# yu45020/Text_Segmentation_Image_Inpainting

Hardware: AMD Instinct MI355X
Metric: imgs/sec fwd+bwd on 512x512 partial-conv inpaint (higher is better)
Workload: dtype f32 (storage, accumulation, stencils, BatchNorm; matrix products = 6-term exact bf16 split on the bf16 MFMA, fp32-class error); 1 GPU; ImageFill 512x512 partial-conv inpainting train step (fwd+bwd, train-mode BN, L1 loss, grad all-reduce, fused SGD), 32 imgs/GPU, random line/ellipse hole masks; global_batch=32, parallelism=dp1, gemm_products=6, activation_storage=f32

## Files before the change

### text_segmentation_image_inpainting_amd/csrc/dwconv.hip

```cpp
#include "tsii_common.h"
#include "dw_lean_api.h"

#include <stdlib.h>

namespace tsii {

struct DwGeom {
    int n, h, w, c, kh, kw, sh, sw, ph, pw, dh, dw, ho, wo;
};

template <bool K3> struct DwPx { static constexpr int value = K3 ? 2 : 4; };
__device__ __forceinline__ int clampi(int v, int lo, int hi) { return v < lo ? lo : (v > hi ? hi : v); }

template <int W, bool K3>
__global__ __launch_bounds__(256) void dw_fwd_kernel(const float* __restrict__ x, const float* __restrict__ rmask,
                                                     const float* __restrict__ wT, const float* __restrict__ bias,
                                                     const float* __restrict__ denom, const float* __restrict__ keep,
                                                     DwGeom g, float* __restrict__ y) {
    constexpr int DW_PX = DwPx<K3>::value;
    const unsigned CG = (unsigned)(g.c / W);
    const unsigned nxg = (unsigned)((g.wo + DW_PX - 1) / DW_PX);
    const unsigned gx = (nxg * CG + 255u) / 256u;
    const unsigned b = xcd_remap(blockIdx.x, gridDim.x);
    const unsigned j = (b % gx) * blockDim.x + threadIdx.x;
// ... 681 lines not shown
            a.w = fmaf(vAA.w, wAA.w, fmaf(vAB.w, wAB.w, fmaf(vBA.w, wBA.w, vBB.w * wBB.w)));
            const float pmk = pls[ty * TW + tx];
            a.x = pmk != 0.f ? a.x * pmk : 0.f; a.y = pmk != 0.f ? a.y * pmk : 0.f;
            a.z = pmk != 0.f ? a.z * pmk : 0.f; a.w = pmk != 0.f ? a.w * pmk : 0.f;
            *reinterpret_cast<float4*>(out_b + (ty * w_in + tx) * c_all) = a;
            if constexpr (BNB) {
                const float4 yq = yv[k];
                const float hx = (yq.x - bmu.x) * bis.x, hy = (yq.y - bmu.y) * bis.y, hz = (yq.z - bmu.z) * bis.z, hw = (yq.w - bmu.w) * bis.w;
                const float zx = fmaf(hx, bga.x, bbe.x), zy = fmaf(hy, bga.y, bbe.y), zz = fmaf(hz, bga.z, bbe.z), zw = fmaf(hw, bga.w, bbe.w);
                const float gx = a.x * ((zx > 0.f && zx < bb.hi) ? 1.f : (zx > 0.f ? 0.f : bb.neg));
                const float gy = a.y * ((zy > 0.f && zy < bb.hi) ? 1.f : (zy > 0.f ? 0.f : bb.neg));
                const float gz = a.z * ((zz > 0.f && zz < bb.hi) ? 1.f : (zz > 0.f ? 0.f : bb.neg));
                const float gw = a.w * ((zw > 0.f && zw < bb.hi) ? 1.f : (zw > 0.f ? 0.f : bb.neg));
                vals[0] += gx; vals[1] += gy; vals[2] += gz; vals[3] += gw;
                vals[4] = fmaf(gx, hx, vals[4]); vals[5] = fmaf(gy, hy, vals[5]);
                vals[6] = fmaf(gz, hz, vals[6]); vals[7] = fmaf(gw, hw, vals[7]);
                if constexpr (DWG) {
                    float4 e = make_float4(0.f, 0.f, 0.f, 0.f);
                    if (pmk != 0.f) {
                        e.x = fminf(fmaxf(zx, zx * bb.neg), bb.hi) * pmk; e.y = fminf(fmaxf(zy, zy * bb.neg), bb.hi) * pmk;
                        e.z = fminf(fmaxf(zz, zz * bb.neg), bb.hi) * pmk; e.w = fminf(fmaxf(zw, zw * bb.neg), bb.hi) * pmk;
                    }
                    dwa[0].x = fmaf(e.x, vAA.x, dwa[0].x); dwa[0].y = fmaf(e.y, vAA.y, dwa[0].y); dwa[0].z = fmaf(e.z, vAA.z, dwa[0].z); dwa[0].w = fmaf(e.w, vAA.w, dwa[0].w);
                    dwa[1].x = fmaf(e.x, vAB.x, dwa[1].x); dwa[1].y = fmaf(e.y, vAB.y, dwa[1].y); dwa[1].z = fmaf(e.z, vAB.z, dwa[1].z); dwa[1].w = fmaf(e.w, vAB.w, dwa[1].w);
                    dwa[2].x = fmaf(e.x, vBA.x, dwa[2].x); dwa[2].y = fmaf(e.y, vBA.y, dwa[2].y); dwa[2].z = fmaf(e.z, vBA.z, dwa[2].z); dwa[2].w = fmaf(e.w, vBA.w, dwa[2].w);
                    dwa[3].x = fmaf(e.x, vBB.x, dwa[3].x); dwa[3].y = fmaf(e.y, vBB.y, dwa[3].y); dwa[3].z = fmaf(e.z, vBB.z, dwa[3].z); dwa[3].w = fmaf(e.w, vBB.w, dwa[3].w);
                }
            }
        }
        lds_barrier();
        if (more) { commit(PRO + NEW * (s + 1), NEW); commit_planes(s + 1); }
        lds_barrier();
    }
    if constexpr (BNB) {
#pragma unroll
        for (int i = 0; i < 8; ++i) {
            float v = vals[i];
            v += __shfl_xor(v, 8, 64); v += __shfl_xor(v, 16, 64); v += __shfl_xor(v, 32, 64);
            vals[i] = v;
        }
        float* mrg = ring;
        if ((threadIdx.x & 63) < CGS) {
#pragma unroll
            for (int i = 0; i < 8; ++i) mrg[((threadIdx.x >> 6) * CGS + cg) * 8 + i] = vals[i];
        }
        __syncthreads();
        if (threadIdx.x < 2 * ST_CB) {
            const int which = threadIdx.x / ST_CB, ch = threadIdx.x % ST_CB;
            if ((int)cb * ST_CB + ch < c_all) {
                float sum = 0.f;
                for (int wv = 0; wv < 4; ++wv) sum += mrg[(wv * CGS + ch / 4) * 8 + which * 4 + ch % 4];
                const int64_t prow = (n * chunks_y + cy) * strips_x + sx;
                bb.part[(prow * 2 + which) * c_all + (int)cb * ST_CB + ch] = sum;
            }
        }
    }
    if constexpr (DWG) {
        float4* m4 = reinterpret_cast<float4*>(dwm);
#pragma unroll
        for (int i = 0; i < 4; ++i) m4[i * 256 + threadIdx.x] = dwa[i];
        __syncthreads();
        const int64_t prow = (n * chunks_y + cy) * strips_x + sx;
        for (int j = threadIdx.x; j < 9 * ST_CB; j += 256) {
            const int tap = j / ST_CB, ch = j % ST_CB;
            if ((int)cb * ST_CB + ch >= c_all) continue;
            const int ky = tap / 3, kx = tap % 3;
            const int slot = (ky == 2 ? 2 : 0) + (kx == 2 ? 1 : 0);
            const int ty_sel = ky == 1 ? 0 : 1, tx_par = kx == 1 ? 0 : 1;
            float sum = 0.f;
#pragma unroll
            for (int l = 0; l < TW / 2; ++l) {
                const int ln = ty_sel * TW + 2 * l + tx_par;
                sum += dwm[((slot * 256 + ln * CGS + ch / 4) * 4) + ch % 4];
            }
            dwpart[(prow * 9 + tap) * c_all + (int)cb * ST_CB + ch] = sum;
        }
    }
}

}
#include "dw_lean.h"
#include "dw_lean_s2.h"
#include "dw_small.h"
#include "dw_rows.h"
namespace tsii {

struct StripPlan {
    bool ok;
    int chunk_rows;
    unsigned strips_x, chunks_y, cblocks;
};
#ifdef TSII_HIP_EMU
static int g_strip_target = 1536;
extern "C" void tsii_emu_set_strip_target(int v) { g_strip_target = v > 0 ? v : 1536; }
#else
#ifndef LS_TARGET
#define LS_TARGET 1536
#endif
static constexpr int g_strip_target = LS_TARGET;
#endif
static StripPlan plan_strip(int n, int hout, int wout, int c, int s, int d) {
    StripPlan p;
    p.ok = ((s == 1 && (d == 1 || d == 2 || d == 4 || d == 8)) || (s == 2 && d == 1)) && c % 4 == 0;
    p.strips_x = cdiv(wout, ST_TW / (s == 2 ? 2 : 1));
    p.cblocks = cdiv(c, ST_CB);
    const int64_t per_chunk = (int64_t)p.strips_x * p.cblocks * n;
    int64_t want = cdiv64(g_strip_target, per_chunk);
    const int max_chunks = cdiv(hout, ST_R);
    if (want > max_chunks) want = max_chunks;
    if (want < 1) want = 1;
    p.chunk_rows = cdiv(cdiv(hout, (int)want), ST_R) * ST_R;
    p.chunks_y = cdiv(hout, p.chunk_rows);
    if (per_chunk * p.chunks_y >= (1ll << 31)) p.ok = false;
    return p;
}

static inline unsigned strip_rows_per_image(const StripPlan& sp) { return sp.ok ? sp.chunks_y * sp.strips_x : 0u; }

struct FusedPlan {
    StripPlan sp;
    unsigned phases;
    bool rows_only;
};
static FusedPlan plan_fwd_strips(int n, int hout, int wout, int c, int s, int d) {
    FusedPlan fp;
    fp.rows_only = false;
    if (dw_phased_dims_ok(hout, wout, c, s, d)) {
        fp.phases = (unsigned)(d * d);
        if ((int64_t)n * d * d < (1ll << 24)) {
            fp.sp = plan_strip(n * d * d, cdiv(hout, d), cdiv(wout, d), c, 1, 1);
            return fp;
        }
    }
    fp.phases = 1u;
    fp.sp = plan_strip(n, hout, wout, c, s, d);
    if (!fp.sp.ok && dw_rows_dims_ok(hout, wout, c, s, d)) {
        fp.sp.ok = true; fp.sp.chunk_rows = hout; fp.sp.strips_x = 1; fp.sp.chunks_y = 1; fp.sp.cblocks = (unsigned)cdiv(c, ST_CB);
        fp.rows_only = true;
    }
    return fp;
}
static inline unsigned fused_rows_per_image(const FusedPlan& fp) { return fp.phases * strip_rows_per_image(fp.sp); }

static const DwBN kNoDwBN = {nullptr, nullptr, 1.f, 0.f};
static const DwBnBwd kNoBnBwd = {nullptr, nullptr, nullptr, nullptr, nullptr, 0.f, 0.f, 0.f, nullptr};

static bool dw_fused_ok(int s, int d) { return (s == 2 && d == 1) || (s == 1 && (d == 1 || d == 2 || d == 4 || d == 8)); }

#ifndef ST_DWG
#define ST_DWG 1
#endif
#ifndef SM_DWG
#define SM_DWG 1
#endif
static bool dw_dxdw_geom_ok(const DtGeom& g) {
    if (g.s != 1 || g.flip != 1 || g.pad_h < 0 || g.pad_w < 0 || g.c % 4 != 0 || dw_rows_ok(g)) return false;
    if (dw_small_ok(g)) return SM_DWG && dw_fused_ok(g.s, g.d);
    if (g.d == 1) return dw_lean_ok(g);
    return ST_DWG && (g.d == 2 || g.d == 4 || g.d == 8);
}

static int try_launch_dw_strip(const float* in, const float* pre, const float* wT, const float* bias, const float* denom,
                               const float* keep, const float* post_mul, DtGeom g, float* out, hipStream_t st,
                               DwBN ib = kNoDwBN, float* stats = nullptr, DwBnBwd bb = kNoBnBwd, float* dwpart = nullptr, bool fold = false) {
    if (g.c % 4 != 0 || !aligned16(in) || !aligned16(out) || !aligned16(wT)) return 1;
    if (ib.sc != nullptr && (!aligned16(ib.sc) || !aligned16(ib.sh))) return 1;
    const FusedPlan fp = plan_fwd_strips(g.n, g.hout, g.wout, g.c, g.s, g.d);
    const StripPlan sp = fp.sp;
    if (dwpart != nullptr && !(dw_dxdw_geom_ok(g) && sp.ok && fp.phases == 1 && !fp.rows_only && bb.y != nullptr && stats == nullptr &&
                               (ib.sc == nullptr) == !fold && denom == nullptr && keep == nullptr && bias == nullptr)) return 1;
    if (fold && dwpart == nullptr) return 1;
    const bool fused_any = ib.sc != nullptr || stats != nullptr || bb.y != nullptr;
    if (dw_rows_ok(g) && pre == nullptr && denom == nullptr && keep == nullptr && post_mul == nullptr && sp.ok &&
        (int64_t)g.n * cdiv(g.c, DR_CB) < (1ll << 31)) {
        const unsigned rcb = (unsigned)cdiv(g.c, DR_CB), rpi = fused_rows_per_image(fp);
        const dim3 rgrid((unsigned)g.n * rcb);
        if (bb.y != nullptr) hipLaunchKernelGGL((dw_rows_kernel<2>), rgrid, dim3(DR_THREADS), 0, st, in, wT, bias, g, rcb, rpi, ib, stats, bb, out);
        else if (fused_any) hipLaunchKernelGGL((dw_rows_kernel<1>), rgrid, dim3(DR_THREADS), 0, st, in, wT, bias, g, rcb, rpi, ib, stats, bb, out);
        else hipLaunchKernelGGL((dw_rows_kernel<0>), rgrid, dim3(DR_THREADS), 0, st, in, wT, bias, g, rcb, rpi, ib, stats, bb, out);
        return check_launch("dw_rows");
    }
    if (fp.rows_only) {
        TSII_REQUIRE(!fused_any, "depth-wise strips: dilation %d has a fused BatchNorm form on the row-phase kernel only (no mask planes, padding = dilation)", g.d);
        return 1;
    }
    if (dw_small_ok(g) && !(post_mul != nullptr && (denom != nullptr || keep != nullptr || bias != nullptr)) && (!fused_any || (sp.ok && dw_fused_ok(g.s, g.d))) &&
        !(fused_any && bb.y == nullptr && post_mul != nullptr)) {
        const bool dxe = denom == nullptr && keep == nullptr && bias == nullptr;
        if (bb.y == nullptr || dxe) {
            const unsigned scb = (unsigned)cdiv(g.c, SM_CB), rpi = sp.ok ? fused_rows_per_image(fp) : 1u;
            const dim3 sgrid((unsigned)g.n * scb);
#define TSII_DW_SMALL(MODE, DXE) do { \
            if (pre != nullptr) hipLaunchKernelGGL((dw_small_kernel<MODE, DXE, true>), sgrid, dim3(SM_THREADS), 0, st, in, pre, wT, bias, denom, keep, post_mul, g, scb, rpi, ib, stats, bb, out); \
            else hipLaunchKernelGGL((dw_small_kernel<MODE, DXE, false>), sgrid, dim3(SM_THREADS), 0, st, in, pre, wT, bias, denom, keep, post_mul, g, scb, rpi, ib, stats, bb, out); } while (0)
            if (bb.y != nullptr && dwpart != nullptr) {
                if (pre != nullptr) hipLaunchKernelGGL((dw_small_kernel<3, true, true>), sgrid, dim3(SM_THREADS), 0, st, in, pre, wT, bias, denom, keep, post_mul, g, scb, rpi, ib, dwpart, bb, out);
                else hipLaunchKernelGGL((dw_small_kernel<3, true, false>), sgrid, dim3(SM_THREADS), 0, st, in, pre, wT, bias, denom, keep, post_mul, g, scb, rpi, ib, dwpart, bb, out);
            }
            else if (bb.y != nullptr) TSII_DW_SMALL(2, true);
            else if (fused_any) TSII_DW_SMALL(1, false);
            else if (dxe) TSII_DW_SMALL(0, true);
            else TSII_DW_SMALL(0, false);
#undef TSII_DW_SMALL
            return check_launch("dw_small");
        }
    }
    if (!sp.ok) return 1;
    const int64_t nblk = (int64_t)sp.strips_x * sp.chunks_y * sp.cblocks * g.n * fp.phases;
    if (nblk >= (1ll << 31)) return fp.phases > 1 ? -1 : 1;
    const dim3 grid((unsigned)nblk);
    const bool fused = ib.sc != nullptr || stats != nullptr || bb.y != nullptr;
    if (!dw_fused_ok(g.s, g.d)) {
        TSII_REQUIRE(!fused, "depth-wise strips: dilation %d has a fused BatchNorm form on the row-phase kernel only (no mask planes, padding = dilation)", g.d);
        return 1;
    }
    if (bb.y != nullptr && g.s != 1) return 1;
    if (fp.phases > 1) {
        const bool takes = dw_lean_phased_ok(g) && !(post_mul != nullptr && (denom != nullptr || keep != nullptr || bias != nullptr));
        const bool dxe = denom == nullptr && keep == nullptr && bias == nullptr;
        if (!takes || (bb.y != nullptr && !dxe) || (fused && bb.y == nullptr && post_mul != nullptr)) {
            TSII_REQUIRE(!fused, "depth-wise strips: this dilated geometry has no fused BatchNorm form (input more than 2 d larger than the output per side?)");
            return 1;
        }
#define TSII_DW_LEAN_PH(MODE, DXE) do { \
            if (pre != nullptr) hipLaunchKernelGGL((dw_lean_kernel<MODE, DXE, true, true>), grid, dim3(256), 0, st, in, pre, wT, bias, denom, keep, post_mul, g, \
                                                   sp.chunk_rows, sp.strips_x, sp.chunks_y, sp.cblocks, ib, stats, bb, out); \
            else hipLaunchKernelGGL((dw_lean_kernel<MODE, DXE, false, true>), grid, dim3(256), 0, st, in, pre, wT, bias, denom, keep, post_mul, g, \
                                    sp.chunk_rows, sp.strips_x, sp.chunks_y, sp.cblocks, ib, stats, bb, out); } while (0)
        if (bb.y != nullptr) TSII_DW_LEAN_PH(2, true);
        else if (fused) TSII_DW_LEAN_PH(1, false);
        else if (dxe) TSII_DW_LEAN_PH(0, true);
        else TSII_DW_LEAN_PH(0, false);
#undef TSII_DW_LEAN_PH
        return check_launch("dw_lean_phased");
    }
    if (dw_lean_ok(g) && !(post_mul != nullptr && (denom != nullptr || keep != nullptr || bias != nullptr))) {
        const bool dxe = denom == nullptr && keep == nullptr && bias == nullptr;
#define TSII_DW_LEAN(MODE, DXE) do { \
            if (pre != nullptr) hipLaunchKernelGGL((dw_lean_kernel<MODE, DXE, true>), grid, dim3(256), 0, st, in, pre, wT, bias, denom, keep, post_mul, g, \
                                                   sp.chunk_rows, sp.strips_x, sp.chunks_y, sp.cblocks, ib, stats, bb, out); \
            else hipLaunchKernelGGL((dw_lean_kernel<MODE, DXE, false>), grid, dim3(256), 0, st, in, pre, wT, bias, denom, keep, post_mul, g, \
                                    sp.chunk_rows, sp.strips_x, sp.chunks_y, sp.cblocks, ib, stats, bb, out); } while (0)
        if (bb.y != nullptr) {
            if (!dxe) return 1;
            if (dwpart != nullptr && fold) {
                if (pre != nullptr) hipLaunchKernelGGL((dw_lean_kernel<4, true, true>), grid, dim3(256), 0, st, in, pre, wT, bias, denom, keep, post_mul, g,
                                                       sp.chunk_rows, sp.strips_x, sp.chunks_y, sp.cblocks, ib, dwpart, bb, out);
                else hipLaunchKernelGGL((dw_lean_kernel<4, true, false>), grid, dim3(256), 0, st, in, pre, wT, bias, denom, keep, post_mul, g,
                                        sp.chunk_rows, sp.strips_x, sp.chunks_y, sp.cblocks, ib, dwpart, bb, out);
                return check_launch("dw_lean (BatchNorm backward on load + dX + dW)");
            }
            if (dwpart != nullptr) {
                if (pre != nullptr) hipLaunchKernelGGL((dw_lean_kernel<3, true, true>), grid, dim3(256), 0, st, in, pre, wT, bias, denom, keep, post_mul, g,
                                                       sp.chunk_rows, sp.strips_x, sp.chunks_y, sp.cblocks, ib, dwpart, bb, out);
                else hipLaunchKernelGGL((dw_lean_kernel<3, true, false>), grid, dim3(256), 0, st, in, pre, wT, bias, denom, keep, post_mul, g,
                                        sp.chunk_rows, sp.strips_x, sp.chunks_y, sp.cblocks, ib, dwpart, bb, out);
                return check_launch("dw_lean (dX + dW)");
            }
            TSII_DW_LEAN(2, true);
        } else if (fused) {
            if (post_mul != nullptr) return 1;
            TSII_DW_LEAN(1, false);
        } else if (dxe) TSII_DW_LEAN(0, true);
        else TSII_DW_LEAN(0, false);
#undef TSII_DW_LEAN
        return check_launch("dw_lean");
    }
    if (dw_lean_s2_ok(g) && post_mul == nullptr && bb.y == nullptr) {
#define TSII_DW_LEAN_S2(MODE) do { \
            if (pre != nullptr) hipLaunchKernelGGL((dw_lean_s2_kernel<MODE, true>), grid, dim3(256), 0, st, in, pre, wT, bias, denom, keep, g, \
                                                   sp.chunk_rows, sp.strips_x, sp.chunks_y, sp.cblocks, ib, stats, out); \
            else hipLaunchKernelGGL((dw_lean_s2_kernel<MODE, false>), grid, dim3(256), 0, st, in, pre, wT, bias, denom, keep, g, \
                                    sp.chunk_rows, sp.strips_x, sp.chunks_y, sp.cblocks, ib, stats, out); } while (0)
        if (fused) TSII_DW_LEAN_S2(1);
        else TSII_DW_LEAN_S2(0);
#undef TSII_DW_LEAN_S2
        return check_launch("dw_lean_s2");
    }
#define TSII_DW_STRIP(S, D, MODE) hipLaunchKernelGGL((dw_strip_kernel<S, D, MODE>), grid, dim3(256), 0, st, in, pre, wT, bias, denom, keep, post_mul, g, \
                                                     sp.chunk_rows, sp.strips_x, sp.chunks_y, sp.cblocks, ib, stats, bb, out)
#define TSII_DW_STRIP_D(D) do { if (bb.y != nullptr && dwpart != nullptr) hipLaunchKernelGGL((dw_strip_kernel<1, D, 3>), grid, dim3(256), 0, st, in, pre, wT, bias, denom, keep, post_mul, g, \
                                                                                          sp.chunk_rows, sp.strips_x, sp.chunks_y, sp.cblocks, ib, dwpart, bb, out); \
                                else if (bb.y != nullptr) TSII_DW_STRIP(1, D, 2); else if (fused) TSII_DW_STRIP(1, D, 1); else TSII_DW_STRIP(1, D, 0); } while (0)
    if (g.s == 2 && fused) TSII_DW_STRIP(2, 1, 1);
    else if (g.s == 2) TSII_DW_STRIP(2, 1, 0);
    else if (g.d == 2) TSII_DW_STRIP_D(2);
    else if (g.d == 4) TSII_DW_STRIP_D(4);
    else if (g.d == 8) TSII_DW_STRIP_D(8);
    else if (bb.y != nullptr) hipLaunchKernelGGL((dw_strip_kernel<1, 1, 2>), grid, dim3(256), 0, st, in, pre, wT, bias, denom, keep, post_mul, g,
                                                 sp.chunk_rows, sp.strips_x, sp.chunks_y, sp.cblocks, ib, stats, bb, out);
    else if (fused) hipLaunchKernelGGL((dw_strip_kernel<1, 1, 1>), grid, dim3(256), 0, st, in, pre, wT, bias, denom, keep, post_mul, g,
                                       sp.chunk_rows, sp.strips_x, sp.chunks_y, sp.cblocks, ib, stats, bb, out);
    else hipLaunchKernelGGL((dw_strip_kernel<1, 1, 0>), grid, dim3(256), 0, st, in, pre, wT, bias, denom, keep, post_mul, g,
                            sp.chunk_rows, sp.strips_x, sp.chunks_y, sp.cblocks, ib, stats, bb, out);
    return check_launch("dw_strip");
}

#ifdef TSII_HIP_EMU
static int g_hdw_lean = 0;
extern "C" void tsii_emu_set_hdw_lean(int v) { g_hdw_lean = v; }
#define HDW_LEAN g_hdw_lean
#else
#ifndef HDW_LEAN
#define HDW_LEAN 0
#endif
#endif
bool hdw_lean_ok(int hout, int wout, int c, int s, int d) {
    if (!HDW_LEAN || !LS_ENABLE || s != 1 || c % 8 != 0 || hout < 1 || wout < 1) return false;
    if (d == 1) {
        const int64_t wmax = (int64_t)wout + 2, hmax = (int64_t)hout + 2;
        return c < (1 << 24) && hmax * wmax * 4 < (1ll << 24) && hmax * wmax * c * 4 < (1ll << 32) && (LS_ROWS * wmax + 64) * c * 4 < (1ll << 31);
    }
    if (!(d == 2 || d == 4) || wout < 8 * d || hout < 4 * d) return false;
    const int64_t wmax = (int64_t)wout + 2 * d, hmax = (int64_t)hout + 2 * d;
    return c < (1 << 24) && hmax * wmax * 4 < (1ll << 24) && hmax * wmax * c * 4 < (1ll << 32) && (LS_ROWS * wmax + 64) * c * 4 * d < (1ll << 31);
}
static FusedPlan hdw_lean_plan(int n, int hout, int wout, int c, int d) {
    FusedPlan fp;
    fp.rows_only = false;
    fp.phases = (unsigned)(d * d);
    fp.sp = plan_strip(n * d * d, cdiv(hout, d), cdiv(wout, d), c, 1, 1);
    return fp;
}
int64_t hdw_lean_rows(int n, int hout, int wout, int c, int s, int d) {
    if (!hdw_lean_ok(hout, wout, c, s, d) || (int64_t)n * d * d >= (1ll << 24)) return 0;
    const FusedPlan fp = hdw_lean_plan(n, hout, wout, c, d);
    return fp.sp.ok ? (int64_t)n * fused_rows_per_image(fp) : 0;
}
int launch_hdw_lean(const void* in, const float* w, const float* bias, int n, int hin, int win, int c, int d, int pad_h, int pad_w,
                    int hout, int wout, int flip, const float* in_sc, const float* in_sh, float in_neg, float in_hi, float* stats,
                    const void* bn_y, const float* bn_mean, const float* bn_var, const float* bn_gamma, const float* bn_beta,
                    float bn_eps, float bn_neg, float bn_hi, float* bn_part, void* out, hipStream_t st) {
    if (hdw_lean_rows(n, hout, wout, c, 1, d) <= 0) return 1;
    if (win > wout + 2 * d || hin > hout + 2 * d || pad_h < 0 || pad_w < 0) return 1;
    DtGeom g = {n, hin, win, c, 1, d, pad_h, pad_w, hout, wout, flip};
    const FusedPlan fp = hdw_lean_plan(n, hout, wout, c, d);
    const StripPlan sp = fp.sp;
    const int64_t nblk = (int64_t)sp.strips_x * sp.chunks_y * sp.cblocks * n * fp.phases;
    if (nblk >= (1ll << 31)) return 1;
    const dim3 grid((unsigned)nblk);
    const DwBN ib = {in_sc, in_sh, in_neg, in_hi};
    const DwBnBwd bb = {reinterpret_cast<const float*>(bn_y), bn_mean, bn_var, bn_gamma, bn_beta, bn_eps, bn_neg, bn_hi, bn_part};
    const float* inf = reinterpret_cast<const float*>(in);
    float* outf = reinterpret_cast<float*>(out);
    const float* none = nullptr;
#define TSII_HDW_LEAN(MODE, DXE, PHV) hipLaunchKernelGGL((dw_lean_kernel<MODE, DXE, false, PHV, true>), grid, dim3(256), 0, st, inf, none, w, bias, none, none, none, g, \
                                                         sp.chunk_rows, sp.strips_x, sp.chunks_y, sp.cblocks, ib, stats, bb, outf)
    if (bn_y != nullptr) { if (d > 1) TSII_HDW_LEAN(2, true, true); else TSII_HDW_LEAN(2, true, false); }
    else if (in_sc != nullptr || stats != nullptr) { if (d > 1) TSII_HDW_LEAN(1, false, true); else TSII_HDW_LEAN(1, false, false); }
    else { if (d > 1) TSII_HDW_LEAN(0, false, true); else TSII_HDW_LEAN(0, false, false); }
// ... 336 lines not shown
    TSII_REQUIRE(dwpart == nullptr, "dw_bwd_dxdw_bn: this geometry has no fused dX + dW form (tsii_dw_bwd_dxdw_ws_bytes() == 0)");
    TSII_REQUIRE(bb.y == nullptr, "dw_bwd_dx_bn: the BatchNorm-backward form needs a marching-strip path (tsii_dw_bwd_stat_rows() > 0)");
    const bool k3 = false;
    const int px = (vec && k3) ? DwPx<true>::value : DwPx<false>::value;
    const int64_t nblk = (int64_t)cdiv(cdiv(wd, px) * (vec ? c / 4 : c), 256) * h * n;
    TSII_REQUIRE(nblk < (1ll << 31), "dw_bwd_dx: grid limit");
    const dim3 grid((unsigned)nblk);
    if (vec && k3) hipLaunchKernelGGL((dw_bwd_dx_kernel<4, true>), grid, dim3(256), 0, st, dy, inv, ws, rmask, g, dx);
    else if (vec) hipLaunchKernelGGL((dw_bwd_dx_kernel<4, false>), grid, dim3(256), 0, st, dy, inv, ws, rmask, g, dx);
    else hipLaunchKernelGGL((dw_bwd_dx_kernel<1, false>), grid, dim3(256), 0, st, dy, inv, ws, rmask, g, dx);
    return check_launch("dw_bwd_dx");
}

extern "C" int tsii_dw_bwd_dx(const float* dy, const float* inv, const float* w, const float* rmask,
                              int n, int h, int wd, int c, int kh, int kw, int sh, int sw, int ph, int pw,
                              int dh, int dw, int ho, int wo, float* dx, float* ws, void* stream) {
    return dw_bwd_dx_impl(dy, inv, w, rmask, n, h, wd, c, kh, kw, sh, sw, ph, pw, dh, dw, ho, wo, kNoBnBwd, dx, ws, stream);
}

extern "C" int tsii_dw_bwd_dx_bn(const float* dy, const float* inv, const float* w, const float* rmask,
                                 int n, int h, int wd, int c, int kh, int kw, int sh, int sw, int ph, int pw,
                                 int dh, int dw, int ho, int wo,
                                 const float* bn_y, const float* bn_mean, const float* bn_var, const float* bn_gamma,
                                 const float* bn_beta, float bn_eps, int bn_act, float bn_slope,
                                 float* dx, float* bwd_part, float* ws, void* stream) {
    TSII_REQUIRE(bn_y && bn_mean && bn_var && bn_gamma && bn_beta && bwd_part, "dw_bwd_dx_bn: null pointer");
    TSII_REQUIRE(aligned16(bn_y) && aligned16(bn_mean) && aligned16(bn_var) && aligned16(bn_gamma) && aligned16(bn_beta),
                 "dw_bwd_dx_bn: BatchNorm operands must be 16-byte aligned");
    InBN tmp;
    TSII_REQUIRE(make_in_bn(bn_mean, bn_var, bn_act, bn_slope, &tmp) == 0, "dw_bwd_dx_bn: activation %d has no load-time form", bn_act);
    const DwBnBwd bb = {bn_y, bn_mean, bn_var, bn_gamma, bn_beta, bn_eps, tmp.neg, tmp.hi, bwd_part};
    return dw_bwd_dx_impl(dy, inv, w, rmask, n, h, wd, c, kh, kw, sh, sw, ph, pw, dh, dw, ho, wo, bb, dx, ws, stream);
}

extern "C" size_t tsii_dw_bwd_dxdw_ws_bytes(int n, int h, int wd, int c, int kh, int kw, int sh, int sw, int ph, int pw, int dh, int dw) {
    if (n <= 0 || h <= 0 || wd <= 0 || c <= 0 || c % 4 != 0 || !(kh == 3 && kw == 3 && dh == dw && dh >= 1)) return 0;
    if (sh == 2 && sw == 2 && ph == 1 && pw == 1 && dh == 1) {
        const StripPlan sp = plan_strip(n, h, wd, c, 1, 1);
        const int64_t rows = (int64_t)n * strip_rows_per_image(sp);
        if (!sp.ok || rows <= 0 || rows >= (1ll << 31) || (int64_t)sp.strips_x * sp.chunks_y * sp.cblocks * n >= (1ll << 31)) return 0;
        return (size_t)rows * 9 * (size_t)c * sizeof(float);
    }
    if (sh != 1 || sw != 1) return 0;
    const int d = dh;
    if (ph < 0 || pw < 0 || ph > 2 * d || pw > 2 * d) return 0;
    const int ho = h + 2 * ph - 2 * d, wo = wd + 2 * pw - 2 * d;
    if (ho <= 0 || wo <= 0) return 0;
    const DtGeom tg = {n, ho, wo, c, 1, d, 2 * d - ph, 2 * d - pw, h, wd, 1};
    if (!dw_dxdw_geom_ok(tg)) return 0;
    const FusedPlan fp = plan_fwd_strips(n, h, wd, c, 1, d);
    if (!fp.sp.ok || fp.phases != 1 || fp.rows_only) return 0;
    const int64_t rows = (int64_t)n * fused_rows_per_image(fp);
    if (rows <= 0 || rows >= (1ll << 31)) return 0;
    return (size_t)rows * 9 * (size_t)c * sizeof(float);
}

extern "C" int tsii_dw_bwd_dxdw_bn(const float* dy, const float* inv, const float* w, const float* rmask,
                                   int n, int h, int wd, int c, int kh, int kw, int sh, int sw, int ph, int pw,
                                   int dh, int dw, int ho, int wo,
                                   const float* bn_y, const float* bn_mean, const float* bn_var, const float* bn_gamma,
                                   const float* bn_beta, float bn_eps, int bn_act, float bn_slope,
                                   float* dx, float* bwd_part, float* dwgt, float* ws, void* ws_dw, size_t ws_dw_bytes, void* stream) {
    TSII_REQUIRE(bn_y && bn_mean && bn_var && bn_gamma && bn_beta && bwd_part && dwgt && ws_dw, "dw_bwd_dxdw_bn: null pointer");
    TSII_REQUIRE(aligned16(bn_y) && aligned16(bn_mean) && aligned16(bn_var) && aligned16(bn_gamma) && aligned16(bn_beta) && aligned16(ws_dw),
                 "dw_bwd_dxdw_bn: BatchNorm operands and the workspace must be 16-byte aligned");
    const size_t need = tsii_dw_bwd_dxdw_ws_bytes(n, h, wd, c, kh, kw, sh, sw, ph, pw, dh, dw);
    TSII_REQUIRE(need > 0, "dw_bwd_dxdw_bn: this geometry has no fused dX + dW form (tsii_dw_bwd_dxdw_ws_bytes() == 0)");
    TSII_REQUIRE(ws_dw_bytes >= need, "dw_bwd_dxdw_bn: weight-gradient workspace too small");
    InBN tmp;
    TSII_REQUIRE(make_in_bn(bn_mean, bn_var, bn_act, bn_slope, &tmp) == 0, "dw_bwd_dxdw_bn: activation %d has no load-time form", bn_act);
    const DwBnBwd bb = {bn_y, bn_mean, bn_var, bn_gamma, bn_beta, bn_eps, tmp.neg, tmp.hi, bwd_part};
    int rc = dw_bwd_dx_impl(dy, inv, w, rmask, n, h, wd, c, kh, kw, sh, sw, ph, pw, dh, dw, ho, wo, bb, dx, ws, stream, (float*)ws_dw);
    if (rc) return rc;
    const int rows = (int)(need / ((size_t)9 * c * sizeof(float)));
    hipLaunchKernelGGL(dw_reduce_kernel, dim3((unsigned)cdiv64((int64_t)9 * c, 32)), dim3(256), 0, (hipStream_t)stream, (const float*)ws_dw, rows, 9, c, dwgt,
                       (float*)nullptr, 9);
    return check_launch("dw_reduce");
}

extern "C" int tsii_dw_bwd_dxdw_fold_ok(int n, int h, int wd, int c, int kh, int kw, int sh, int sw, int ph, int pw, int dh, int dw) {
#ifndef DX2_FOLD
#define DX2_FOLD 1
#endif
    return (sh == sw && (sh == 1 || (DX2_FOLD && sh == 2)) && dh == 1 && dw == 1 && tsii_dw_bwd_dxdw_ws_bytes(n, h, wd, c, kh, kw, sh, sw, ph, pw, dh, dw) > 0) ? 1 : 0;
}

extern "C" int tsii_dw_bwd_dxdw_bn2(const float* da2, const float* bn2_y, const float* bn2_coef, int bn2_act, float bn2_slope,
                                    const float* inv, const float* w, const float* rmask,
                                    int n, int h, int wd, int c, int kh, int kw, int sh, int sw, int ph, int pw,
                                    int dh, int dw, int ho, int wo,
                                    const float* bn_y, const float* bn_mean, const float* bn_var, const float* bn_gamma,
                                    const float* bn_beta, float bn_eps, int bn_act, float bn_slope,
                                    float* dx, float* bwd_part, float* dwgt, float* ws, void* ws_dw, size_t ws_dw_bytes, void* stream) {
    TSII_REQUIRE(da2 && bn2_y && bn2_coef && bn_y && bn_mean && bn_var && bn_gamma && bn_beta && bwd_part && dwgt && ws_dw, "dw_bwd_dxdw_bn2: null pointer");
    TSII_REQUIRE(aligned16(bn_y) && aligned16(bn_mean) && aligned16(bn_var) && aligned16(bn_gamma) && aligned16(bn_beta) && aligned16(ws_dw) &&
                 aligned16(bn2_y) && aligned16(da2), "dw_bwd_dxdw_bn2: tensors and the workspace must be 16-byte aligned");
    TSII_REQUIRE(tsii_dw_bwd_dxdw_fold_ok(n, h, wd, c, kh, kw, sh, sw, ph, pw, dh, dw), "dw_bwd_dxdw_bn2: this geometry has no form with the BatchNorm backward on load");
    const size_t need = tsii_dw_bwd_dxdw_ws_bytes(n, h, wd, c, kh, kw, sh, sw, ph, pw, dh, dw);
    TSII_REQUIRE(ws_dw_bytes >= need, "dw_bwd_dxdw_bn2: weight-gradient workspace too small");
    InBN tmp, tmp2;
    TSII_REQUIRE(make_in_bn(bn_mean, bn_var, bn_act, bn_slope, &tmp) == 0, "dw_bwd_dxdw_bn2: activation %d has no load-time form", bn_act);
    TSII_REQUIRE(make_in_bn(bn2_y, bn2_coef, bn2_act, bn2_slope, &tmp2) == 0, "dw_bwd_dxdw_bn2: activation %d has no load-time form", bn2_act);
    const DwBnBwd bb = {bn_y, bn_mean, bn_var, bn_gamma, bn_beta, bn_eps, tmp.neg, tmp.hi, bwd_part};
    const DwBN fold_ib = {bn2_y, bn2_coef, tmp2.neg, tmp2.hi};
    int rc = dw_bwd_dx_impl(da2, inv, w, rmask, n, h, wd, c, kh, kw, sh, sw, ph, pw, dh, dw, ho, wo, bb, dx, ws, stream, (float*)ws_dw, fold_ib);
    if (rc) return rc;
    const int rows = (int)(need / ((size_t)9 * c * sizeof(float)));
    hipLaunchKernelGGL(dw_reduce_kernel, dim3((unsigned)cdiv64((int64_t)9 * c, 32)), dim3(256), 0, (hipStream_t)stream, (const float*)ws_dw, rows, 9, c, dwgt,
                       (float*)nullptr, 9);
    return check_launch("dw_reduce");
}

extern "C" size_t tsii_dw_bwd_dw_ws_bytes(int n, int ho, int wo, int c, int kh, int kw) {
    if (n <= 0 || ho <= 0 || wo <= 0 || c <= 0 || kh <= 0 || kw <= 0) return 0;
    const DwPlan a = plan_dw(n, ho, c, c % 4 == 0), b = plan_dw(n, ho, c, false);
    int R = a.R > b.R ? a.R : b.R;
    if (kh == 3 && kw == 3) {
        for (int ss = 1; ss <= 2; ++ss) {
            const StripPlan sp = plan_strip(n, ho, wo, c, ss, 1);
            const int64_t g2 = (int64_t)n * sp.chunks_y * sp.strips_x;
            if (g2 > R) R = (int)g2;
        }
    }
    return (size_t)R * (size_t)(kh * kw + 1) * c * sizeof(float);
}

static int dw_bwd_dw_impl(const float* dy, const float* inv, const float* keep, const float* x, const float* rmask,
                          int n, int h, int wd, int c, int kh, int kw, int sh, int sw, int ph, int pw,
                          int dh, int dw, int ho, int wo, DwBN ib, float* dwgt, float* dbias, void* ws, size_t ws_bytes,
                          void* stream) {
    TSII_REQUIRE(dy && x && dwgt && ws, "dw_bwd_dw: null pointer");
    DW_GEOM();
    if (check_geom(g, "dw_bwd_dw")) return -1;
    TSII_REQUIRE(ws_bytes >= tsii_dw_bwd_dw_ws_bytes(n, ho, wo, c, kh, kw), "dw_bwd_dw: workspace too small");
    hipStream_t st = (hipStream_t)stream;
    const bool vec = (c % 4 == 0) && aligned16(dy) && aligned16(x) && (ib.sc == nullptr || (aligned16(ib.sc) && aligned16(ib.sh)));
    float* part = (float*)ws;
    if (vec && kh == 3 && kw == 3 && sh == 1 && sw == 1 && dh == dw && inv == nullptr && keep == nullptr && rmask == nullptr) {
        DtGeom rg = {n, h, wd, c, 1, dh, ph, pw, ho, wo, 0};
        if (dw_rows_ok(rg) && (int64_t)n * cdiv(c, DR_CB) < (1ll << 31)) {
            const unsigned rcb = (unsigned)cdiv(c, DR_CB);
            if (ib.sc != nullptr) hipLaunchKernelGGL((dw_rows_dw_kernel<true>), dim3((unsigned)n * rcb), dim3(DR_THREADS), 0, st, dy, x, rg, rcb, ib, part);
            else hipLaunchKernelGGL((dw_rows_dw_kernel<false>), dim3((unsigned)n * rcb), dim3(DR_THREADS), 0, st, dy, x, rg, rcb, ib, part);
            int rc0 = check_launch("dw_rows_dw");
            if (rc0) return rc0;
            hipLaunchKernelGGL(dw_reduce_kernel, dim3((unsigned)cdiv64((int64_t)10 * c, 32)), dim3(256), 0, st, part, n, 9, c, dwgt, dbias, 0);
            return check_launch("dw_reduce");
        }
    }
    if (vec && kh == 3 && kw == 3 && sh == sw && dh == dw &&
        ((sh == 1 && (dh == 1 || dh == 2 || dh == 4 || dh == 8)) || (sh == 2 && dh == 1))) {
        const StripPlan sp = plan_strip(n, ho, wo, c, sh, dh);
        if (sp.ok) {
            DtGeom tg = {n, h, wd, c, sh, dh, ph, pw, ho, wo, 0};
            const unsigned rows = (unsigned)n * sp.chunks_y * sp.strips_x;
            const dim3 grid(rows * sp.cblocks);
            if (sh == 2) hipLaunchKernelGGL((dw_strip_dw_kernel<2, 1>), grid, dim3(256), 0, st, dy, inv, keep, x, rmask, tg, sp.chunk_rows,
                                            sp.strips_x, sp.chunks_y, sp.cblocks, ib, part);
            else if (dh == 1) hipLaunchKernelGGL((dw_strip_dw_kernel<1, 1>), grid, dim3(256), 0, st, dy, inv, keep, x, rmask, tg, sp.chunk_rows,
                                                 sp.strips_x, sp.chunks_y, sp.cblocks, ib, part);
            else if (dh == 4) hipLaunchKernelGGL((dw_strip_dw_kernel<1, 4>), grid, dim3(256), 0, st, dy, inv, keep, x, rmask, tg, sp.chunk_rows,
                                                 sp.strips_x, sp.chunks_y, sp.cblocks, ib, part);
            else if (dh == 8) hipLaunchKernelGGL((dw_strip_dw_kernel<1, 8>), grid, dim3(256), 0, st, dy, inv, keep, x, rmask, tg, sp.chunk_rows,
                                                 sp.strips_x, sp.chunks_y, sp.cblocks, ib, part);
            else hipLaunchKernelGGL((dw_strip_dw_kernel<1, 2>), grid, dim3(256), 0, st, dy, inv, keep, x, rmask, tg, sp.chunk_rows,
                                    sp.strips_x, sp.chunks_y, sp.cblocks, ib, part);
// ... 40 lines not shown
```

Before: 565.9 imgs/s.

## Add whole-map LDS depthwise kernel for small dilated maps with fused BN backward

Adds a depthwise 3x3 kernel for small dilated stride-1 maps (up to 32x32) that stages the whole spatial map for 16 channels in LDS with zero-padded border slots. It serves forward, fused BN-stats, BN-backward, dX+dW and the folded BN-backward-on-load modes in one launch per image and channel block. It also lets the fold path accept dilated geometries. The aim is to replace the strip or small-kernel paths, which handle dilated taps and per-strip overhead poorly on tiny feature maps. The cost is register pressure, shared-memory use that limits occupancy to two blocks per CU, and new dispatch checks.

```diff
diff --git a/text_segmentation_image_inpainting_amd/csrc/dw_map.h b/text_segmentation_image_inpainting_amd/csrc/dw_map.h
--- /dev/null
+++ b/text_segmentation_image_inpainting_amd/csrc/dw_map.h
@@ -0,0 +1,272 @@
+#pragma once
+
+namespace tsii {
+
+#ifndef DW_MAP
+#define DW_MAP 1
+#endif
+#ifndef DM_MIN_DIL
+#define DM_MIN_DIL 2
+#endif
+static constexpr int DM_CB = 16;
+static constexpr int DM_SIDE = 32;
+static constexpr int DM_PIX = (DM_SIDE + 1) * (DM_SIDE + 1);
+static constexpr int DM_THREADS = 256;
+static constexpr int DM_LANES = DM_THREADS / 4;
+static constexpr int DM_NP = DM_SIDE * DM_SIDE / DM_LANES;
+
+static inline bool dw_map_ok(const DtGeom& g) {
+    return DW_MAP && g.s == 1 && g.d >= DM_MIN_DIL && g.hin == g.hout && g.win == g.wout && g.pad_h == g.d && g.pad_w == g.d &&
+           g.hin <= DM_SIDE && g.win <= DM_SIDE && (g.hin * g.win) % DM_LANES == 0 && g.c % 4 == 0 && g.c < (1 << 24) && (int64_t)g.hin * g.win * g.c * 4 < (1ll << 31);
+}
+
+template <int MODE, bool DXE, bool PRE>
+__global__ __launch_bounds__(DM_THREADS, 2) void dw_map_kernel(
+    const float* __restrict__ in, const float* __restrict__ pre, const float* __restrict__ wT, const float* __restrict__ bias,
+    const float* __restrict__ denom, const float* __restrict__ keep, const float* __restrict__ post_mul, DtGeom g,
+    unsigned cblocks, unsigned rows_per_image, DwBN ib, float* __restrict__ stats, DwBnBwd bb, float* __restrict__ out) {
+    constexpr bool FUSED = (MODE == 1), BNB = (MODE >= 2), DWG = (MODE >= 3), APL = (MODE == 4);
+    static_assert(!BNB || DXE, "K6c rides on the dX epilogue");
+    static_assert(!FUSED || !DXE, "K6b rides on the forward epilogue");
+    static_assert(2 * DM_PIX * DM_CB * sizeof(float) <= 160 * 1024, "two blocks per CU");
+    __shared__ __attribute__((aligned(16))) float tile[DM_PIX * DM_CB];
+    const unsigned b = xcd_remap(blockIdx.x, gridDim.x);
+    const unsigned cb = b % cblocks;
+    const int64_t n = b / cblocks;
+    const int t = threadIdx.x;
+    const int cq = t & 3, lane = t >> 2;
+    const int C = g.c, H = g.hin, W = g.win, HW = H * W, D = g.d;
+    const int c0 = (int)cb * DM_CB + cq * 4;
+    const bool cok = c0 < C;
+    const unsigned c0b = (unsigned)(cok ? c0 : C - 4) * 4u;
+    const char* const ibase = reinterpret_cast<const char*>(in + n * HW * (int64_t)C);
+    const char* const y2base = reinterpret_cast<const char*>(APL ? ib.sc + n * HW * (int64_t)C : nullptr);
+    const float* const pbase = pre + (PRE ? n * HW : 0);
+    auto opq = [](unsigned o) { TSII_OPAQUE_U32(o); return o; };
+    const unsigned wmagic = (unsigned)(((1 << 20) + W - 1) / W);
+
+    f32x4 pf[DM_NP];
+    f32x4 pf2[APL ? DM_NP : 1];
+    float pm[DM_NP];
+#pragma unroll
+    for (int j = 0; j < DM_NP; ++j) {
+        if (j * DM_LANES >= HW) break;
+        const unsigned pc = (unsigned)(lane + DM_LANES * j);
+        const unsigned off = opq(__umul24(pc * 4u, (unsigned)C) + c0b);
+        pf[j] = *reinterpret_cast<const f32x4*>(ibase + off);
+        if (APL) pf2[j] = *reinterpret_cast<const f32x4*>(y2base + off);
+        pm[j] = PRE ? pbase[pc] : 1.f;
+    }
+    f32x4 isc = {1.f, 1.f, 1.f, 1.f}, ish = {0.f, 0.f, 0.f, 0.f}, bq = {0.f, 0.f, 0.f, 0.f};
+    const bool has_bn = FUSED && ib.sc != nullptr;
+    if (has_bn && cok) { isc = *reinterpret_cast<const f32x4*>(ib.sc + c0); ish = *reinterpret_cast<const f32x4*>(ib.sh + c0); }
+    if (!DXE && bias != nullptr && cok) bq = *reinterpret_cast<const f32x4*>(bias + c0);
+    const float bn_neg = has_bn ? ib.neg : 1.f;
+    const bool hi_finite = has_bn && ib.hi < __builtin_huge_valf();
+    char* const lthr = reinterpret_cast<char*>(tile) + cq * 16;
+    {
+        f32x4 amu = {0.f, 0.f, 0.f, 0.f}, ais = amu, aga = amu, abe = amu, ak1 = amu, ak2 = amu;
+        if (APL && cok) {
+            const float* cf = ib.sh + c0;
+            amu = *reinterpret_cast<const f32x4*>(cf); ais = *reinterpret_cast<const f32x4*>(cf + C);
+            aga = *reinterpret_cast<const f32x4*>(cf + 2 * (int64_t)C); abe = *reinterpret_cast<const f32x4*>(cf + 3 * (int64_t)C);
+            ak1 = *reinterpret_cast<const f32x4*>(cf + 4 * (int64_t)C); ak2 = *reinterpret_cast<const f32x4*>(cf + 5 * (int64_t)C);
+        }
+#pragma unroll
+        for (int j = 0; j < DM_NP; ++j) {
+            if (j * DM_LANES >= HW) break;
+            const int p = lane + DM_LANES * j;
+            f32x4 v = pf[j];
+            if (FUSED) {
+                f32x2 z0 = fma2(v.xy, isc.xy, ish.xy), z1 = fma2(v.zw, isc.zw, ish.zw);
+                z0 = max2(z0, z0 * bn_neg); z1 = max2(z1, z1 * bn_neg);
+                if (hi_finite) { z0 = min2(z0, f32x2{ib.hi, ib.hi}); z1 = min2(z1, f32x2{ib.hi, ib.hi}); }
+                v = cat4(z0, z1);
+            }
+            if (APL) {
+                const f32x4 y2 = pf2[APL ? j : 0];
+                const f32x2 h0 = (y2.xy - amu.xy) * ais.xy, h1 = (y2.zw - amu.zw) * ais.zw;
+                const f32x2 z0 = fma2(h0, aga.xy, abe.xy), z1 = fma2(h1, aga.zw, abe.zw);
+                f32x2 d0 = v.xy, d1 = v.zw;
+                d0.x *= (z0.x > 0.f && z0.x < ib.hi) ? 1.f : (z0.x > 0.f ? 0.f : ib.neg);
+                d0.y *= (z0.y > 0.f && z0.y < ib.hi) ? 1.f : (z0.y > 0.f ? 0.f : ib.neg);
+                d1.x *= (z1.x > 0.f && z1.x < ib.hi) ? 1.f : (z1.x > 0.f ? 0.f : ib.neg);
+                d1.y *= (z1.y > 0.f && z1.y < ib.hi) ? 1.f : (z1.y > 0.f ? 0.f : ib.neg);
+                d0 = (d0 - ak1.xy) - h0 * ak2.xy; d1 = (d1 - ak1.zw) - h1 * ak2.zw;
+                v = cat4((d0 * aga.xy) * ais.xy, (d1 * aga.zw) * ais.zw);
+            }
+            v *= pm[j];
+            const int y = (int)(((unsigned)p * wmagic) >> 20);
+            *reinterpret_cast<f32x4*>(lthr + (p + y) * (DM_CB * 4)) = v;
+        }
+    }
+    for (int i = t; i < (H + W + 1) * 4; i += DM_THREADS) {
+        const int q = i >> 2;
+        const int zp = q < H ? q * (W + 1) + W : H * (W + 1) + (q - H);
+        *reinterpret_cast<f32x4*>(reinterpret_cast<char*>(tile) + (zp * 4 + (i & 3)) * 16) = f32x4{0.f, 0.f, 0.f, 0.f};
+    }
+    f32x4 w[9];
+#pragma unroll
+    for (int k = 0; k < 9; ++k) w[k] = cok ? *reinterpret_cast<const f32x4*>(wT + (g.flip ? 8 - k : k) * C + c0) : f32x4{0.f, 0.f, 0.f, 0.f};
+    f32x4 bmu = {0.f, 0.f, 0.f, 0.f}, bis = bmu, bga = bmu, bbe = bmu;
+    if (BNB && cok) {
+        bmu = *reinterpret_cast<const f32x4*>(bb.mean + c0);
+        const f32x4 vr = *reinterpret_cast<const f32x4*>(bb.var + c0);
+        bis = f32x4{1.0f / sqrtf(vr.x + bb.eps), 1.0f / sqrtf(vr.y + bb.eps), 1.0f / sqrtf(vr.z + bb.eps), 1.0f / sqrtf(vr.w + bb.eps)};
+        bga = *reinterpret_cast<const f32x4*>(bb.gamma + c0);
+        bbe = *reinterpret_cast<const f32x4*>(bb.beta + c0);
+    }
+    const char* const ybase = reinterpret_cast<const char*>(BNB ? bb.y + n * HW * (int64_t)C : nullptr);
+    const float* const dpl = denom != nullptr ? denom + n * HW : nullptr;
+    const float* const kpl = keep != nullptr ? keep + n * HW : nullptr;
+    const float* const qpl = post_mul != nullptr ? post_mul + n * HW : nullptr;
+    f32x4 yvr[BNB ? DM_NP : 1];
+    float ep0[DM_NP], ep1[DXE ? 1 : DM_NP];
+#pragma unroll
+    for (int j = 0; j < DM_NP; ++j) {
+        if (j * DM_LANES >= HW) break;
+        const unsigned pc = (unsigned)(lane + DM_LANES * j);
+        if (BNB) yvr[BNB ? j : 0] = *reinterpret_cast<const f32x4*>(ybase + opq(__umul24(pc * 4u, (unsigned)C) + c0b));
+        if (DXE) ep0[j] = qpl != nullptr ? qpl[pc] : 1.f;
+        else { ep0[j] = dpl != nullptr ? dpl[pc] : 1.f; ep1[DXE ? 0 : j] = kpl != nullptr ? kpl[pc] : 1.f; }
+    }
+    __syncthreads();
+
+    const char* const rthr = reinterpret_cast<const char*>(tile) + cq * 16;
+    char* const obase = reinterpret_cast<char*>(out + n * HW * (int64_t)C);
+    const int PB = (W + 1) * (DM_CB * 4);
+    f32x4 P = {0.f, 0.f, 0.f, 0.f};
+    f32x2 va[4] = {f32x2{0.f, 0.f}, f32x2{0.f, 0.f}, f32x2{0.f, 0.f}, f32x2{0.f, 0.f}};
+    int cnt = 0;
+    f32x4 dwa[DWG ? 9 : 1];
+#pragma unroll
+    for (int k = 0; k < (DWG ? 9 : 1); ++k) dwa[k] = f32x4{0.f, 0.f, 0.f, 0.f};
+#pragma unroll
+    for (int j = 0; j < DM_NP; ++j) {
+        if (j * DM_LANES >= HW) break;
+        const int p = lane + DM_LANES * j;
+        const bool pok = cok;
+        const int y = (int)(((unsigned)p * wmagic) >> 20), x = p - y * W;
+        const float e0 = ep0[j], e1 = DXE ? 1.f : ep1[DXE ? 0 : j];
+        const f32x4 yv = BNB ? yvr[BNB ? j : 0] : f32x4{0.f, 0.f, 0.f, 0.f};
+        f32x4 ein = {0.f, 0.f, 0.f, 0.f};
+        if (DWG && pok && e0 != 0.f) {
+            const f32x2 g0 = fma2((yv.xy - bmu.xy) * bis.xy, bga.xy, bbe.xy), g1 = fma2((yv.zw - bmu.zw) * bis.zw, bga.zw, bbe.zw);
+            const f32x2 q0 = min2(max2(g0, g0 * bb.neg), f32x2{bb.hi, bb.hi}) * e0, q1 = min2(max2(g1, g1 * bb.neg), f32x2{bb.hi, bb.hi}) * e0;
+            ein = cat4(q0, q1);
+        }
+        int rb[3], cx[3];
+        rb[0] = (y - D >= 0 ? y - D : H) * PB; rb[1] = y * PB; rb[2] = (y + D < H ? y + D : H) * PB;
+        cx[0] = (x - D >= 0 ? x - D : W) * (DM_CB * 4); cx[1] = x * (DM_CB * 4); cx[2] = (x + D < W ? x + D : W) * (DM_CB * 4);
+        f32x2 a0 = {0.f, 0.f}, a1 = {0.f, 0.f};
+#pragma unroll
+        for (int ky = 0; ky < 3; ++ky) {
+#pragma unroll
+            for (int kx = 0; kx < 3; ++kx) {
+                const f32x4 v = *reinterpret_cast<const f32x4*>(rthr + rb[ky] + cx[kx]);
+                a0 = fma2(v.xy, w[ky * 3 + kx].xy, a0);
+                a1 = fma2(v.zw, w[ky * 3 + kx].zw, a1);
+                if (DWG) {
+                    f32x4& q = dwa[DWG ? ky * 3 + kx : 0];
+                    q = cat4(fma2(v.xy, ein.xy, q.xy), fma2(v.zw, ein.zw, q.zw));
+                }
+            }
+        }
+        if (DXE) {
+            a0 *= e0; a1 *= e0;
+            if (e0 == 0.f) { a0 = f32x2{0.f, 0.f}; a1 = a0; }
+        } else {
+            const float r = 1.0f / e0;
+            a0 *= r; a1 *= r;
+            a0 += bq.xy; a1 += bq.zw;
+            if (e1 == 0.f) { a0 = f32x2{0.f, 0.f}; a1 = a0; }
+        }
+        if (pok) {
+            __builtin_nontemporal_store(cat4(a0, a1), reinterpret_cast<f32x4*>(obase + opq(__umul24((unsigned)p * 4u, (unsigned)C) + (unsigned)c0 * 4u)));
+            if (FUSED) {
+                if (cnt == 0) P = cat4(a0, a1);
+                const f32x2 d0 = a0 - P.xy, d1 = a1 - P.zw;
+                va[0] += d0; va[1] += d1;
+                va[2] = fma2(d0, d0, va[2]); va[3] = fma2(d1, d1, va[3]);
+                ++cnt;
+            }
+            if (BNB) {
+                const f32x2 h0 = (yv.xy - bmu.xy) * bis.xy, h1 = (yv.zw - bmu.zw) * bis.zw;
+                const f32x2 z0 = fma2(h0, bga.xy, bbe.xy), z1 = fma2(h1, bga.zw, bbe.zw);
+                f32x2 d0 = a0, d1 = a1;
+                d0.x *= (z0.x > 0.f && z0.x < bb.hi) ? 1.f : (z0.x > 0.f ? 0.f : bb.neg);
+                d0.y *= (z0.y > 0.f && z0.y < bb.hi) ? 1.f : (z0.y > 0.f ? 0.f : bb.neg);
+                d1.x *= (z1.x > 0.f && z1.x < bb.hi) ? 1.f : (z1.x > 0.f ? 0.f : bb.neg);
+                d1.y *= (z1.y > 0.f && z1.y < bb.hi) ? 1.f : (z1.y > 0.f ? 0.f : bb.neg);
+                va[0] += d0; va[1] += d1;
+                va[2] = fma2(d0, h0, va[2]); va[3] = fma2(d1, h1, va[3]);
+            }
+        }
+    }
+    if (!(BNB || (FUSED && stats != nullptr))) return;
+    __syncthreads();
+    float* mrg = tile;
+    float* mt = mrg + t * 13;
+    mt[0] = (float)cnt;
+    mt[1] = P.x; mt[2] = P.y; mt[3] = P.z; mt[4] = P.w;
+    mt[5] = va[0].x; mt[6] = va[0].y; mt[7] = va[1].x; mt[8] = va[1].y;
+    mt[9] = va[2].x; mt[10] = va[2].y; mt[11] = va[3].x; mt[12] = va[3].y;
+    __syncthreads();
+    if (BNB) {
+        if (t < 2 * DM_CB) {
+            const int which = t / DM_CB, ch = t % DM_CB;
+            if ((int)cb * DM_CB + ch < C) {
+                float sum = 0.f;
+                for (int l = 0; l < DM_LANES; ++l) sum += mrg[(l * 4 + ch / 4) * 13 + 5 + which * 4 + ch % 4];
+                bb.part[(n * rows_per_image * 2 + which) * C + (int)cb * DM_CB + ch] = sum;
+                for (unsigned r = 1; r < rows_per_image; ++r) bb.part[((n * rows_per_image + r) * 2 + which) * C + (int)cb * DM_CB + ch] = 0.f;
+            }
+        }
+        if (DWG) {
+            static_assert(9 * DM_THREADS * 16 <= DM_PIX * DM_CB * 4, "weight-gradient merge buffer fits the tile");
+            f32x4* m4 = reinterpret_cast<f32x4*>(tile);
+            __syncthreads();
+#pragma unroll
+            for (int k = 0; k < 9; ++k) m4[k * DM_THREADS + t] = dwa[DWG ? k : 0];
+            __syncthreads();
+            if (t < 9 * DM_CB) {
+                const int k = t / DM_CB, ch = t % DM_CB;
+                if ((int)cb * DM_CB + ch < C) {
+                    const float* col = tile + (k * DM_THREADS + ch / 4) * 4 + ch % 4;
+                    float sum = 0.f;
+#pragma unroll 8
+                    for (int l = 0; l < DM_LANES; ++l) sum += col[l * 16];
+                    const int tap = g.flip ? 8 - k : k;
+                    stats[((n * rows_per_image) * 9 + tap) * C + (int)cb * DM_CB + ch] = sum;
+                    for (unsigned r = 1; r < rows_per_image; ++r) stats[((n * rows_per_image + r) * 9 + tap) * C + (int)cb * DM_CB + ch] = 0.f;
+                }
+            }
+        }
+    } else if (t < DM_CB && (int)cb * DM_CB + t < C) {
+        const int ch = t, mcg = ch / 4, mi = ch % 4;
+        float nn = 0.f, pv = 0.f, s1 = 0.f, s2 = 0.f;
+        bool have = false;
+        {
+            const float* qi = mrg + (33 * 4 + mcg) * 13;
+            if (qi[0] != 0.f) { pv = qi[1 + mi]; have = true; }
+        }
+        for (int l = 0; l < DM_LANES; ++l) {
+            const float* q = mrg + (l * 4 + mcg) * 13;
+            const float n_t = q[0];
+            if (n_t == 0.f) continue;
+            if (!have) { pv = q[1 + mi]; have = true; }
+            const float dp = q[1 + mi] - pv, b1 = q[5 + mi], b2 = q[9 + mi];
+            s1 += fmaf(n_t, dp, b1);
+            s2 += b2 + dp * (2.f * b1 + n_t * dp);
+            nn += n_t;
+        }
+        float* sp = stats + n * rows_per_image * 4 * C + (int)cb * DM_CB + ch;
+        sp[0] = nn;
+        sp[C] = pv;
+        sp[2 * (int64_t)C] = s1;
+        sp[3 * (int64_t)C] = s2;
+        for (unsigned r = 1; r < rows_per_image; ++r) sp[(int64_t)r * 4 * C] = 0.f;
+    }
+}
+
+}
diff --git a/text_segmentation_image_inpainting_amd/csrc/dwconv.hip b/text_segmentation_image_inpainting_amd/csrc/dwconv.hip
--- a/text_segmentation_image_inpainting_amd/csrc/dwconv.hip
+++ b/text_segmentation_image_inpainting_amd/csrc/dwconv.hip
@@ -787,6 +787,7 @@
 #include "dw_lean.h"
 #include "dw_lean_s2.h"
 #include "dw_small.h"
+#include "dw_map.h"
 #include "dw_rows.h"
 namespace tsii {
 
@@ -860,6 +861,7 @@
 #endif
 static bool dw_dxdw_geom_ok(const DtGeom& g) {
     if (g.s != 1 || g.flip != 1 || g.pad_h < 0 || g.pad_w < 0 || g.c % 4 != 0 || dw_rows_ok(g)) return false;
+    if (dw_map_ok(g)) return dw_fused_ok(g.s, g.d);
     if (dw_small_ok(g)) return SM_DWG && dw_fused_ok(g.s, g.d);
     if (g.d == 1) return dw_lean_ok(g);
     return ST_DWG && (g.d == 2 || g.d == 4 || g.d == 8);
@@ -889,6 +891,27 @@
         TSII_REQUIRE(!fused_any, "depth-wise strips: dilation %d has a fused BatchNorm form on the row-phase kernel only (no mask planes, padding = dilation)", g.d);
         return 1;
     }
+    if (dw_map_ok(g) && !(post_mul != nullptr && (denom != nullptr || keep != nullptr || bias != nullptr)) && (!fused_any || (sp.ok && dw_fused_ok(g.s, g.d))) &&
+        !(fused_any && bb.y == nullptr && post_mul != nullptr)) {
+        const bool dxe = denom == nullptr && keep == nullptr && bias == nullptr;
+        if (bb.y == nullptr || dxe) {
+            const unsigned mcb = (unsigned)cdiv(g.c, DM_CB), rpi = sp.ok ? fused_rows_per_image(fp) : 1u;
+            const dim3 mgrid((unsigned)g.n * mcb);
+#define TSII_DW_MAP(MODE, DXE, ST) do { \
+            if (pre != nullptr) hipLaunchKernelGGL((dw_map_kernel<MODE, DXE, true>), mgrid, dim3(DM_THREADS), 0, st, in, pre, wT, bias, denom, keep, post_mul, g, mcb, rpi, ib, ST, bb, out); \
+            else hipLaunchKernelGGL((dw_map_kernel<MODE, DXE, false>), mgrid, dim3(DM_THREADS), 0, st, in, pre, wT, bias, denom, keep, post_mul, g, mcb, rpi, ib, ST, bb, out); } while (0)
+            if (bb.y != nullptr && dwpart != nullptr && fold) TSII_DW_MAP(4, true, dwpart);
+            else if (bb.y != nullptr && dwpart != nullptr) TSII_DW_MAP(3, true, dwpart);
+            else if (bb.y != nullptr) TSII_DW_MAP(2, true, stats);
+            else if (fused_any) TSII_DW_MAP(1, false, stats);
+            else if (dxe) TSII_DW_MAP(0, true, stats);
+            else TSII_DW_MAP(0, false, stats);
+#undef TSII_DW_MAP
+            return check_launch("dw_map");
+        }
+    }
+    TSII_REQUIRE(!fold || (g.d == 1 && dw_lean_ok(g) && fp.phases == 1),
+                 "dw_bwd_dxdw_bn2: this geometry has no form with the BatchNorm backward on load (tsii_dw_bwd_dxdw_fold_ok() == 0)");
     if (dw_small_ok(g) && !(post_mul != nullptr && (denom != nullptr || keep != nullptr || bias != nullptr)) && (!fused_any || (sp.ok && dw_fused_ok(g.s, g.d))) &&
         !(fused_any && bb.y == nullptr && post_mul != nullptr)) {
         const bool dxe = denom == nullptr && keep == nullptr && bias == nullptr;
@@ -971,6 +994,7 @@
 #undef TSII_DW_LEAN
         return check_launch("dw_lean");
     }
+    TSII_REQUIRE(!fold, "dw_bwd_dxdw_bn2: this geometry has no form with the BatchNorm backward on load (tsii_dw_bwd_dxdw_fold_ok() == 0)");
     if (dw_lean_s2_ok(g) && post_mul == nullptr && bb.y == nullptr) {
 #define TSII_DW_LEAN_S2(MODE) do { \
             if (pre != nullptr) hipLaunchKernelGGL((dw_lean_s2_kernel<MODE, true>), grid, dim3(256), 0, st, in, pre, wT, bias, denom, keep, g, \
@@ -1473,6 +1497,11 @@
 #ifndef DX2_FOLD
 #define DX2_FOLD 1
 #endif
+    if (sh == 1 && sw == 1 && dh == dw && dh > 1) {
+        if (n <= 0 || h <= 0 || wd <= 0 || c <= 0 || ph != dh || pw != dw) return 0;
+        const DtGeom tg = {n, h, wd, c, 1, dh, dh, dw, h, wd, 1};
+        return (dw_map_ok(tg) && tsii_dw_bwd_dxdw_ws_bytes(n, h, wd, c, kh, kw, sh, sw, ph, pw, dh, dw) > 0) ? 1 : 0;
+    }
     return (sh == sw && (sh == 1 || (DX2_FOLD && sh == 2)) && dh == 1 && dw == 1 && tsii_dw_bwd_dxdw_ws_bytes(n, h, wd, c, kh, kw, sh, sw, ph, pw, dh, dw) > 0) ? 1 : 0;
 }
 
```

After: 570.8 imgs/s, median of 6. No clear change (+0.9%).
